# hyx1999/SAM-Decoding

Measured on AMD Instinct MI355X. Metric: tokens/sec (+ mean accepted tokens), Vicuna-7B bs=1, samd_sam_only draft+verify, higher is better.
Workload: dtype f16

## Files before the change

### sam-decoding_amd/csrc/verify_kernels.hip

```cpp
#include <hip/hip_runtime.h>
#include <hip/hip_fp16.h>
#include <cstdlib>
#include <cstring>
#include <vector>
#include "samd_common.h"
#include "topk_device.h"
#include "warm_device.h"

#define HIPCHK(x) do { hipError_t e_ = (x); if (e_ != hipSuccess) { samd_set_error("%s: %s", #x, hipGetErrorString(e_)); return SAMD_E_HIP; } } while (0)
#define LAUNCHCHK() do { hipError_t e_ = hipGetLastError(); if (e_ != hipSuccess) { samd_set_error("kernel launch: %s", hipGetErrorString(e_)); return SAMD_E_HIP; } } while (0)

typedef _Float16 half8 __attribute__((ext_vector_type(8)));
typedef __bf16 bf16x8 __attribute__((ext_vector_type(8)));
typedef float floatx4 __attribute__((ext_vector_type(4)));

struct F16 { typedef _Float16 elem; typedef half8 vec8; };
struct BF16 { typedef __bf16 elem; typedef bf16x8 vec8; };

__device__ __forceinline__ float to_f32(_Float16 x) { return (float)x; }
__device__ __forceinline__ float to_f32(__bf16 x) { return (float)x; }
__device__ __forceinline__ float to_f32(float x) { return x; }

template <typename T>
__global__ __launch_bounds__(1024) void k_argmax_rows(const T *__restrict__ logits, int rows, long long vocab, long long stride,
                                                      const int *__restrict__ d_rows, int *__restrict__ out) {
    const int row = blockIdx.x;
    if (d_rows && row >= d_rows[0]) return;
    if (row >= rows) return;
    const T *x = logits + (size_t)row * stride;
    float best = -INFINITY; long long bi = 0x7fffffffffffffffll;
    constexpr int VEC = 16 / sizeof(T);
    const bool vec_ok = ((((size_t)x) & 15) == 0);
    const long long nvec = vec_ok ? vocab / VEC : 0;
    for (long long c = threadIdx.x; c < nvec; c += blockDim.x) {
        const uint4 raw = reinterpret_cast<const uint4 *>(x)[c];
        const T *e = reinterpret_cast<const T *>(&raw);
#pragma unroll
        for (int j = 0; j < VEC; j++) {
            const float v = to_f32(e[j]); const long long i = c * VEC + j;
            if (v > best || (v == best && i < bi)) { best = v; bi = i; }
        }
    }
    for (long long i = nvec * VEC + threadIdx.x; i < vocab; i += blockDim.x) {
        const float v = to_f32(x[i]);
        if (v > best || (v == best && i < bi)) { best = v; bi = i; }
    }
    for (int o = 32; o > 0; o >>= 1) {
        const float ov = __shfl_xor(best, o); const long long oi = __shfl_xor(bi, o);
        if (ov > best || (ov == best && oi < bi)) { best = ov; bi = oi; }
    }
    __shared__ float sv[16]; __shared__ long long si[16];
    const int w = threadIdx.x >> 6;
    if ((threadIdx.x & 63) == 0) { sv[w] = best; si[w] = bi; }
    __syncthreads();
    if (threadIdx.x == 0) {
        const int nw = blockDim.x >> 6;
        for (int k = 1; k < nw; k++) if (sv[k] > best || (sv[k] == best && si[k] < bi)) { best = sv[k]; bi = si[k]; }
        out[row] = (bi == 0x7fffffffffffffffll) ? 0 : (int)bi;
    }
}

__global__ __launch_bounds__(256) void k_kv_compact(void *const *__restrict__ tensors, const int *__restrict__ verdict,
                                                    const int *__restrict__ kv_index, int n_heads, long long max_len, int row_bytes,
                                                    int h_start, int h_accept, int n_row_major) {
    extern __shared__ __attribute__((aligned(16))) unsigned char smem[];
    int a = h_accept, start = h_start;
    if (verdict) {
        if (!verdict[V_IS_TREE]) return;
        a = verdict[V_ACCEPT]; start = verdict[V_KV_START];
    }
    const int t = blockIdx.x / n_heads;
    unsigned char *base = (unsigned char *)tensors[t] + (size_t)(blockIdx.x % n_heads) * max_len * row_bytes;
    if (t >= n_row_major) {
        const int D = row_bytes >> 1, total = a * D;
        unsigned short *lds = reinterpret_cast<unsigned short *>(smem);
        unsigned short *col = reinterpret_cast<unsigned short *>(base);
        for (int c = threadIdx.x; c < total; c += blockDim.x) {
            const int d = c / a, j = c - d * a;
            lds[c] = col[(size_t)d * max_len + start + kv_index[j]];
        }
        __syncthreads();
        for (int c = threadIdx.x; c < total; c += blockDim.x) {
            const int d = c / a, j = c - d * a;
            if (kv_index[j] == j) continue;
            col[(size_t)d * max_len + start + j] = lds[c];
        }
        return;
    }
    const int chunks = row_bytes >> 4, total = a * chunks;
    uint4 *lds = reinterpret_cast<uint4 *>(smem);
    for (int c = threadIdx.x; c < total; c += blockDim.x) {
        const int j = c / chunks, k = c - j * chunks;
        const long long src = (long long)start + kv_index[j];
        lds[c] = reinterpret_cast<const uint4 *>(base + (size_t)src * row_bytes)[k];
    }
    __syncthreads();
    for (int c = threadIdx.x; c < total; c += blockDim.x) {
        const int j = c / chunks, k = c - j * chunks;
        if (kv_index[j] == j) continue;
        reinterpret_cast<uint4 *>(base + (size_t)(start + j) * row_bytes)[k] = lds[c];
    }
}

#define ATT_TILE 64
#define ATT_SPLITS 16
#define ATT_D 128
#define VT_STRIDE (ATT_TILE + 8)
#define P_STRIDE (ATT_TILE + 8)

template <typename TT> struct Mfma;
template <> struct Mfma<F16> {
    static __device__ __forceinline__ floatx4 run(half8 a, half8 b, floatx4 c) { return __builtin_amdgcn_mfma_f32_16x16x32_f16(a, b, c, 0, 0, 0); }
};
template <> struct Mfma<BF16> {
    static __device__ __forceinline__ floatx4 run(bf16x8 a, bf16x8 b, floatx4 c) { return __builtin_amdgcn_mfma_f32_16x16x32_bf16(a, b, c, 0, 0, 0); }
};

__device__ __forceinline__ int att_head_of_block(int bx, int n_heads) {
    return (n_heads & 7) == 0 ? (bx & 7) * (n_heads >> 3) + (bx >> 3) : bx;
}

template <typename TT, bool WIDE, bool VT = false>
__global__ __launch_bounds__(256) void k_tree_attention(const typename TT::elem *__restrict__ q, const typename TT::elem *__restrict__ kc,
                                                        const typename TT::elem *__restrict__ vc, float *__restrict__ ws,
                                                        int n_q_pad, int n_heads, int n_kv_heads, long long max_len,
                                                        const unsigned long long *__restrict__ mask, const int *__restrict__ d_L,
                                                        const int *__restrict__ d_n, float scale_log2, WarmArgs warm) {
    typedef typename TT::elem E;
    typedef typename TT::vec8 V8;
    __shared__ __attribute__((aligned(16))) E Vt[ATT_D * VT_STRIDE];
    __shared__ __attribute__((aligned(16))) E Pw[4 * 16 * P_STRIDE];

    const int h = att_head_of_block(blockIdx.x, n_heads), split = blockIdx.y;
    if (split >= ATT_SPLITS) {
        if (blockIdx.z != 0) return;
        const unsigned a = warm_next_projection(warm, (split - ATT_SPLITS) * n_heads + h);
        if (a == 0x9E3779B9u && n_q_pad < 0) ws[0] = 0.f;
        return;
    }
    const int tid = threadIdx.x, w = tid >> 6, l = tid & 63, lr = l & 15, lg = l >> 4;
    const int row_base = (WIDE ? 64 * (int)blockIdx.z : 0) + 16 * w;
    V8 qa[4];
    {
        const int qrow = row_base + lr;
        const E *qp = q + ((size_t)qrow * n_heads + h) * ATT_D + 8 * lg;
#pragma unroll
        for (int kk = 0; kk < 4; kk++) {
            uint4 raw = make_uint4(0, 0, 0, 0);
            if (qrow < n_q_pad) raw = *reinterpret_cast<const uint4 *>(qp + 32 * kk);
            qa[kk] = __builtin_bit_cast(V8, raw);
        }
    }
    unsigned long long mrow[4], mrow_hi[WIDE ? 4 : 1];
#pragma unroll
    for (int r = 0; r < 4; r++) {
        mrow[r] = mask[row_base + 4 * lg + r];
        if constexpr (WIDE) mrow_hi[r] = mask[SAMD_MAX_DRAFT + row_base + 4 * lg + r];
    }
    const int kvh = h / (n_heads / n_kv_heads);
    const E *kbase = kc + (size_t)kvh * max_len * ATT_D;
    const E *vbase = vc + (size_t)kvh * max_len * ATT_D;
    const bool may_be_active = row_base < n_q_pad;
    uint4 kraw[4][4], vra[2], vrb[2];
    auto load_k = [&](int key0) {
#pragma unroll
        for (int st = 0; st < 4; st++) {
            int key = key0 + 16 * st + lr;
// ... 3 lines not shown
            for (int kk = 0; kk < 4; kk++) kraw[st][kk] = *reinterpret_cast<const uint4 *>(kp + 32 * kk);
        }
    };
    auto load_v = [&](int key0) {
        if constexpr (VT) {
#pragma unroll
            for (int i = 0; i < 4; i++) {
                const int u = tid + 256 * i, d = u >> 3;
                int k0 = key0 + 8 * (u & 7);
                k0 = k0 + 8 <= (int)max_len ? k0 : (int)max_len - 8;
                const uint4 v = *reinterpret_cast<const uint4 *>(vbase + (size_t)d * max_len + k0);
                if (i == 0) vra[0] = v; else if (i == 1) vra[1] = v; else if (i == 2) vrb[0] = v; else vrb[1] = v;
            }
            return;
        }
#pragma unroll
        for (int it = 0; it < 2; it++) {
            const int p = tid >> 3, ch = (tid & 7) + 8 * it, d0 = 8 * ch;
            int ka = key0 + 2 * p, kb = ka + 1;
            ka = ka < (int)max_len ? ka : (int)max_len - 1; kb = kb < (int)max_len ? kb : (int)max_len - 1;
            vra[it] = *reinterpret_cast<const uint4 *>(vbase + (size_t)ka * ATT_D + d0);
            vrb[it] = *reinterpret_cast<const uint4 *>(vbase + (size_t)kb * ATT_D + d0);
        }
    };
    if (may_be_active) load_k(split * ATT_TILE);
    load_v(split * ATT_TILE);
    const int L = d_L[0];
    int n = d_n[0]; n = n > n_q_pad ? n_q_pad : n;
    const int total = L + n;
    const int ntiles = (total + ATT_TILE - 1) / ATT_TILE;
    if (split >= ntiles) return;
    const bool active = row_base < n;
#pragma unroll
    for (int r = 0; r < 4; r++) if (row_base + 4 * lg + r >= n) { mrow[r] = 0ull; if constexpr (WIDE) mrow_hi[r] = 0ull; }

    float m_run[4], l_run[4];
    floatx4 o[8];
#pragma unroll
    for (int r = 0; r < 4; r++) { m_run[r] = -INFINITY; l_run[r] = 0.f; }
#pragma unroll
    for (int dt = 0; dt < 8; dt++) o[dt] = (floatx4){0.f, 0.f, 0.f, 0.f};

    E *Pmine = Pw + w * 16 * P_STRIDE;

    for (int t = split; t < ntiles; t += ATT_SPLITS) {
        const int key0 = t * ATT_TILE;
        if (t != split && active) load_k(key0);
        __syncthreads();
        if (t != split) load_v(key0);
        if constexpr (VT) {
#pragma unroll
            for (int i = 0; i < 4; i++) {
                const int u = tid + 256 * i, d = u >> 3, kc8 = 8 * (u & 7);
                uint4 v = i == 0 ? vra[0] : (i == 1 ? vra[1] : (i == 2 ? vrb[0] : vrb[1]));
                const int live = total - key0 - kc8;
                if (live < 8) {
                    unsigned m[4];
#pragma unroll
                    for (int d2 = 0; d2 < 4; d2++) m[d2] = (2 * d2 < live ? 0xFFFFu : 0u) | (2 * d2 + 1 < live ? 0xFFFF0000u : 0u);
                    v.x &= m[0]; v.y &= m[1]; v.z &= m[2]; v.w &= m[3];
                }
                *reinterpret_cast<uint4 *>(&Vt[d * VT_STRIDE + kc8]) = v;
            }
        } else
#pragma unroll
        for (int it = 0; it < 2; it++) {
            const int p = tid >> 3, ch = (tid & 7) + 8 * it, d0 = 8 * ch;
            const int ka = key0 + 2 * p, kb = ka + 1;
            const uint4 ra = ka < total ? vra[it] : make_uint4(0, 0, 0, 0), rb = kb < total ? vrb[it] : make_uint4(0, 0, 0, 0);
            const unsigned short *ea = reinterpret_cast<const unsigned short *>(&ra);
            const unsigned short *eb = reinterpret_cast<const unsigned short *>(&rb);
#pragma unroll
            for (int j = 0; j < 8; j++)
                *reinterpret_cast<unsigned int *>(&Vt[(d0 + j) * VT_STRIDE + 2 * p]) = (unsigned int)ea[j] | ((unsigned int)eb[j] << 16);
        }
        floatx4 s[4];
        if (active) {
#pragma unroll
            for (int st = 0; st < 4; st++) {
                floatx4 acc = (floatx4){0.f, 0.f, 0.f, 0.f};
#pragma unroll
                for (int kk = 0; kk < 4; kk++) acc = Mfma<TT>::run(qa[kk], __builtin_bit_cast(V8, kraw[st][kk]), acc);
                s[st] = acc;
            }
            float tmax[4];
#pragma unroll
            for (int r = 0; r < 4; r++) tmax[r] = -INFINITY;
#pragma unroll
            for (int st = 0; st < 4; st++) {
                const int key = key0 + 16 * st + lr;
#pragma unroll
                for (int r = 0; r < 4; r++) {
                    const int rel = key - L;
                    bool ok;
                    if constexpr (WIDE) {
                        const unsigned long long word = rel < 64 ? mrow[r] : mrow_hi[r];
                        ok = (key < L) | ((key < total) & (bool)((word >> (rel & 63)) & 1ull));
                    } else ok = (key < L) | ((key < total) & (bool)((mrow[r] >> (rel & 63)) & 1ull));
                    const float v = ok ? s[st][r] * scale_log2 : -INFINITY;
                    s[st][r] = v;
                    tmax[r] = fmaxf(tmax[r], v);
                }
            }
#pragma unroll
            for (int r = 0; r < 4; r++) {
                const float v = row16_max(tmax[r]);
                const float m_new = fmaxf(m_run[r], v);
                const float m_use = m_new == -INFINITY ? 0.f : m_new;
                const float alpha = __builtin_amdgcn_exp2f(m_run[r] - m_use);
                float psum = 0.f;
#pragma unroll
                for (int st = 0; st < 4; st++) {
                    const float p = __builtin_amdgcn_exp2f(s[st][r] - m_use);
                    psum += p;
                    Pmine[(4 * lg + r) * P_STRIDE + 16 * st + lr] = (E)p;
                }
                psum = row16_sum(psum);
                l_run[r] = l_run[r] * alpha + psum;
                m_run[r] = m_new;
#pragma unroll
                for (int dt = 0; dt < 8; dt++) o[dt][r] *= alpha;
            }
        }
        __syncthreads();
        if (active) {
            V8 pa[2];
#pragma unroll
            for (int kcx = 0; kcx < 2; kcx++)
                pa[kcx] = __builtin_bit_cast(V8, *reinterpret_cast<const uint4 *>(&Pmine[lr * P_STRIDE + 32 * kcx + 8 * lg]));
#pragma unroll
            for (int dt = 0; dt < 8; dt++) {
#pragma unroll
                for (int kcx = 0; kcx < 2; kcx++) {
                    const uint4 raw = *reinterpret_cast<const uint4 *>(&Vt[(16 * dt + lr) * VT_STRIDE + 32 * kcx + 8 * lg]);
                    o[dt] = Mfma<TT>::run(pa[kcx], __builtin_bit_cast(V8, raw), o[dt]);
                }
            }
        }
    }
    if (active) {
#pragma unroll
        for (int r = 0; r < 4; r++) {
            const int row = row_base + 4 * lg + r;
            float *dst = ws + (((size_t)split * n_q_pad + row) * n_heads + h) * (ATT_D + 2);
            if (row < n_q_pad) {
#pragma unroll
                for (int dt = 0; dt < 8; dt++) dst[16 * dt + lr] = o[dt][r];
                if (lr == 0) { dst[ATT_D] = m_run[r]; dst[ATT_D + 1] = l_run[r]; }
            }
        }
    }
}

template <typename TT>
__global__ __launch_bounds__(64) void k_tree_attention_direct(const typename TT::elem *__restrict__ q, const typename TT::elem *__restrict__ kc,
                                                               const typename TT::elem *__restrict__ vt, float *__restrict__ ws,
                                                               int n_q_pad, int n_heads, int n_kv_heads, long long max_len,
                                                               const unsigned long long *__restrict__ mask, const int *__restrict__ d_L,
                                                               const int *__restrict__ d_n, float scale_log2, WarmArgs warm) {
    typedef typename TT::elem E;
    typedef typename TT::vec8 V8;
    __shared__ __attribute__((aligned(16))) E Pw[16 * P_STRIDE];
    const int h = att_head_of_block(blockIdx.x, n_heads), split = blockIdx.y;
    if (split >= ATT_SPLITS) {
        if (blockIdx.z != 0) return;
        const unsigned a = warm_next_projection(warm, (split - ATT_SPLITS) * n_heads + h);
        if (a == 0x9E3779B9u && n_q_pad < 0) ws[0] = 0.f;
        return;
    }
    const int l = threadIdx.x, lr = l & 15, lg = l >> 4;
    const int row_base = 16 * (int)blockIdx.z;
    V8 qa[4];
    {
        const E *qp = q + ((size_t)(row_base + lr) * n_heads + h) * ATT_D + 8 * lg;
#pragma unroll
        for (int kk = 0; kk < 4; kk++) {
            uint4 raw = make_uint4(0, 0, 0, 0);
            if (row_base + lr < n_q_pad) raw = *reinterpret_cast<const uint4 *>(qp + 32 * kk);
            qa[kk] = __builtin_bit_cast(V8, raw);
        }
    }
    unsigned long long mrow[4];
#pragma unroll
    for (int r = 0; r < 4; r++) mrow[r] = row_base + 4 * lg + r < n_q_pad ? mask[row_base + 4 * lg + r] : 0ull;
    const int kvh = h / (n_heads / n_kv_heads);
    const E *kbase = kc + (size_t)kvh * max_len * ATT_D;
    const E *vbase = vt + (size_t)kvh * max_len * ATT_D;
    uint4 kraw[4][4], vraw[8][2];
    auto load_kv = [&](int key0) {
#pragma unroll
        for (int st = 0; st < 4; st++) {
            int key = key0 + 16 * st + lr;
            key = key < (int)max_len ? key : (int)max_len - 1;
            const E *kp = kbase + (size_t)key * ATT_D + 8 * lg;
#pragma unroll
            for (int kk = 0; kk < 4; kk++) kraw[st][kk] = *reinterpret_cast<const uint4 *>(kp + 32 * kk);
        }
#pragma unroll
        for (int kcx = 0; kcx < 2; kcx++) {
            int k0 = key0 + 32 * kcx + 8 * lg;
            k0 = k0 + 8 <= (int)max_len ? k0 : (int)max_len - 8;
#pragma unroll
            for (int dt = 0; dt < 8; dt++) vraw[dt][kcx] = *reinterpret_cast<const uint4 *>(vbase + (size_t)(16 * dt + lr) * max_len + k0);
        }
    };
    load_kv(split * ATT_TILE);
    const int L = d_L[0];
    int n = d_n[0]; n = n > n_q_pad ? n_q_pad : n;
    const int total = L + n;
    const int ntiles = (total + ATT_TILE - 1) / ATT_TILE;
    if (split >= ntiles || row_base >= n) return;
#pragma unroll
    for (int r = 0; r < 4; r++) if (row_base + 4 * lg + r >= n) mrow[r] = 0ull;
    float m_run[4], l_run[4];
    floatx4 o[8];
#pragma unroll
    for (int r = 0; r < 4; r++) { m_run[r] = -INFINITY; l_run[r] = 0.f; }
#pragma unroll
    for (int dt = 0; dt < 8; dt++) o[dt] = (floatx4){0.f, 0.f, 0.f, 0.f};
    for (int t = split; t < ntiles; t += ATT_SPLITS) {
        const int key0 = t * ATT_TILE;
        if (t != split) load_kv(key0);
        floatx4 s[4];
#pragma unroll
        for (int st = 0; st < 4; st++) {
            floatx4 acc = (floatx4){0.f, 0.f, 0.f, 0.f};
#pragma unroll
            for (int kk = 0; kk < 4; kk++) acc = Mfma<TT>::run(qa[kk], __builtin_bit_cast(V8, kraw[st][kk]), acc);
            s[st] = acc;
        }
        float tmax[4];
#pragma unroll
        for (int r = 0; r < 4; r++) tmax[r] = -INFINITY;
#pragma unroll
        for (int st = 0; st < 4; st++) {
            const int key = key0 + 16 * st + lr;
#pragma unroll
            for (int r = 0; r < 4; r++) {
                const int rel = key - L;
                const bool ok = (key < L) | ((key < total) & (bool)((mrow[r] >> (rel & 63)) & 1ull));
                const float v = ok ? s[st][r] * scale_log2 : -INFINITY;
                s[st][r] = v;
                tmax[r] = fmaxf(tmax[r], v);
            }
        }
        if (t != split) { __builtin_amdgcn_fence(__ATOMIC_RELEASE, "wavefront"); __builtin_amdgcn_wave_barrier(); }
#pragma unroll
        for (int r = 0; r < 4; r++) {
            const float v = row16_max(tmax[r]);
            const float m_new = fmaxf(m_run[r], v);
            const float m_use = m_new == -INFINITY ? 0.f : m_new;
            const float alpha = __builtin_amdgcn_exp2f(m_run[r] - m_use);
            float psum = 0.f;
#pragma unroll
            for (int st = 0; st < 4; st++) {
                const float p = __builtin_amdgcn_exp2f(s[st][r] - m_use);
                psum += p;
                Pw[(4 * lg + r) * P_STRIDE + 16 * st + lr] = (E)p;
            }
            psum = row16_sum(psum);
            l_run[r] = l_run[r] * alpha + psum;
            m_run[r] = m_new;
#pragma unroll
            for (int dt = 0; dt < 8; dt++) o[dt][r] *= alpha;
        }
        if (key0 + ATT_TILE > total) {
#pragma unroll
            for (int kcx = 0; kcx < 2; kcx++) {
                const int live = total - key0 - 32 * kcx - 8 * lg;
                unsigned m[4];
#pragma unroll
                for (int d2 = 0; d2 < 4; d2++) m[d2] = (2 * d2 < live ? 0xFFFFu : 0u) | (2 * d2 + 1 < live ? 0xFFFF0000u : 0u);
#pragma unroll
                for (int dt = 0; dt < 8; dt++) { vraw[dt][kcx].x &= m[0]; vraw[dt][kcx].y &= m[1]; vraw[dt][kcx].z &= m[2]; vraw[dt][kcx].w &= m[3]; }
            }
        }
        __builtin_amdgcn_fence(__ATOMIC_RELEASE, "wavefront"); __builtin_amdgcn_wave_barrier();
        V8 pa[2];
#pragma unroll
        for (int kcx = 0; kcx < 2; kcx++) pa[kcx] = __builtin_bit_cast(V8, *reinterpret_cast<const uint4 *>(&Pw[lr * P_STRIDE + 32 * kcx + 8 * lg]));
#pragma unroll
        for (int dt = 0; dt < 8; dt++) {
#pragma unroll
            for (int kcx = 0; kcx < 2; kcx++) o[dt] = Mfma<TT>::run(pa[kcx], __builtin_bit_cast(V8, vraw[dt][kcx]), o[dt]);
        }
    }
#pragma unroll
    for (int r = 0; r < 4; r++) {
        const int row = row_base + 4 * lg + r;
        float *dst = ws + (((size_t)split * n_q_pad + row) * n_heads + h) * (ATT_D + 2);
        if (row < n) {
#pragma unroll
            for (int dt = 0; dt < 8; dt++) dst[16 * dt + lr] = o[dt][r];
            if (lr == 0) { dst[ATT_D] = m_run[r]; dst[ATT_D + 1] = l_run[r]; }
        }
    }
}

template <typename E>
__global__ __launch_bounds__(128) void k_attn_combine(const float *__restrict__ ws, E *__restrict__ out, int n_q_pad, int n_heads,
                                                      const int *__restrict__ d_L, const int *__restrict__ d_n, WarmArgs warm, int *__restrict__ arrive) {
    const int h = att_head_of_block(blockIdx.x, n_heads), row = blockIdx.y, d = threadIdx.x;
    if (row >= n_q_pad) {
        const unsigned a = warm_next_projection(warm, (row - n_q_pad) * n_heads + h);
        if (a == 0x9E3779B9u && n_q_pad < 0) out[0] = (E)0.f;
        return;
    }
    float mv[ATT_SPLITS], lv[ATT_SPLITS], pv[ATT_SPLITS];
    const int lane = d & 63;
    float2 ml = make_float2(-INFINITY, 0.f);
    if (lane < ATT_SPLITS) ml = *reinterpret_cast<const float2 *>(ws + (((size_t)lane * n_q_pad + row) * n_heads + h) * (ATT_D + 2) + ATT_D);
#pragma unroll
    for (int s = 0; s < ATT_SPLITS; s++) pv[s] = ws[(((size_t)s * n_q_pad + row) * n_heads + h) * (ATT_D + 2) + d];
#pragma unroll
    for (int s = 0; s < ATT_SPLITS; s++) { mv[s] = __shfl(ml.x, s); lv[s] = __shfl(ml.y, s); }
    int n = d_n[0]; n = n > n_q_pad ? n_q_pad : n;
    E *dst = out + ((size_t)row * n_heads + h) * ATT_D + d;
    float res = 0.f;
    if (row < n) {
        const int ntiles = (d_L[0] + n + ATT_TILE - 1) / ATT_TILE;
        const int used = ntiles < ATT_SPLITS ? ntiles : ATT_SPLITS;
        float M = -INFINITY;
#pragma unroll
        for (int s = 0; s < ATT_SPLITS; s++) if (s < used) M = fmaxf(M, mv[s]);
        float num = 0.f, den = 0.f;
#pragma unroll
        for (int s = 0; s < ATT_SPLITS; s++) {
            if (s >= used || mv[s] == -INFINITY) continue;
            const float wgt = exp2f(mv[s] - M);
            num += wgt * pv[s]; den += wgt * lv[s];
        }
        res = den > 0.f ? num / den : 0.f;
    }
    *dst = (E)res;
    if (arrive) {
        __syncthreads();
        if (threadIdx.x == 0) {
            __builtin_amdgcn_fence(__ATOMIC_RELEASE, "agent");
            asm volatile("s_waitcnt vmcnt(0)" ::: "memory");
            __hip_atomic_fetch_add(arrive, 1, __ATOMIC_RELAXED, __HIP_MEMORY_SCOPE_AGENT);
        }
    }
}

#define ATT_SLOTS (ATT_SPLITS + 1)
#define QS_STRIDE (ATT_D + 8)

template <typename TT, int NP>
__global__ __launch_bounds__(256, 2) void k_tree_attention_rope(const typename TT::elem *__restrict__ qkv, int n_part_rt, long long part_stride,
                                                               const float *__restrict__ cs, typename TT::elem *__restrict__ kc,
                                                               typename TT::elem *__restrict__ vc, float *__restrict__ ws,
                                                               int n_q_pad, int n_heads, int n_kv_heads, long long max_len,
                                                               const unsigned long long *__restrict__ mask, const int *__restrict__ d_L,
                                                               const int *__restrict__ d_n, float scale_log2) {
    typedef typename TT::elem E;
    typedef typename TT::vec8 V8;
    __shared__ __attribute__((aligned(16))) E Vt[ATT_D * VT_STRIDE];
    __shared__ __attribute__((aligned(16))) E Pw[4 * 16 * P_STRIDE];
    __shared__ __attribute__((aligned(16))) E Qs[ATT_TILE * QS_STRIDE];

    const int h = blockIdx.x, split = blockIdx.y;
    const bool fresh = split == ATT_SPLITS;
    const int tid = threadIdx.x, w = tid >> 6, l = tid & 63, lr = l & 15, lg = l >> 4;
    const int row_base = 16 * w;
    const int group = n_heads / n_kv_heads, kvh = h / group;
    const int W = (n_heads + 2 * n_kv_heads) * ATT_D;
    const float *part = reinterpret_cast<const float *>(qkv);

    auto ld4 = [&](size_t off, float (&x)[4]) {
        if constexpr (NP == 0) {
            const uint2 raw = *reinterpret_cast<const uint2 *>(qkv + off);
            const E *e = reinterpret_cast<const E *>(&raw);
#pragma unroll
            for (int i = 0; i < 4; i++) x[i] = (float)e[i];
        } else if constexpr (NP > 0) {
            float4 a[NP];
            const unsigned pst = (unsigned)part_stride;
#pragma unroll
            for (int k = 0; k < NP; k++) a[k] = *reinterpret_cast<const float4 *>(part + off + (unsigned)k * pst);
            float acc[4] = {0.f, 0.f, 0.f, 0.f};
#pragma unroll
            for (int k = 0; k < NP; k++) { acc[0] += a[k].x; acc[1] += a[k].y; acc[2] += a[k].z; acc[3] += a[k].w; }
#pragma unroll
            for (int i = 0; i < 4; i++) x[i] = (float)(E)acc[i];
        } else {
            float acc[4] = {0.f, 0.f, 0.f, 0.f};
            for (int k = 0; k < n_part_rt; k++) {
                const float4 a = *reinterpret_cast<const float4 *>(part + (size_t)k * part_stride + off);
                acc[0] += a.x; acc[1] += a.y; acc[2] += a.z; acc[3] += a.w;
            }
#pragma unroll
            for (int i = 0; i < 4; i++) x[i] = (float)(E)acc[i];
        }
    };
    auto rope_units = [&](int rows, int col0, E *dst, bool to_cache, const int *pL, const int *pn) {
        float x1[4][4], x2[4][4];
        float4 c[4], sn[4];
#pragma unroll
        for (int k = 0; k < 4; k++) {
            const int u = tid + 256 * k;
            if (u >= rows * 16) continue;
            const int r = u >> 4, e = 4 * (u & 15);
            ld4((size_t)r * W + col0 + e, x1[k]);
            ld4((size_t)r * W + col0 + e + 64, x2[k]);
            c[k] = *reinterpret_cast<const float4 *>(cs + r * ATT_D + e);
            sn[k] = *reinterpret_cast<const float4 *>(cs + r * ATT_D + 64 + e);
        }
        const int Lw = to_cache ? pL[0] : 0, nn = to_cache ? pn[0] : 0;
#pragma unroll
        for (int k = 0; k < 4; k++) {
            const int u = tid + 256 * k;
            if (u >= rows * 16) continue;
            const int r = u >> 4, e = 4 * (u & 15);
            const float cc[4] = {c[k].x, c[k].y, c[k].z, c[k].w}, ss[4] = {sn[k].x, sn[k].y, sn[k].z, sn[k].w};
            E lo[4], hi[4];
#pragma unroll
            for (int i = 0; i < 4; i++) {
                lo[i] = (E)(x1[k][i] * cc[i] - x2[k][i] * ss[i]);
// ... 394 lines not shown
        bool grown = false;
        while (true) {
            if (tid == 0) {
                int action = 0, tok = -1, hit = -1;
                while (row < C) {
                    const int j = row++;
                    bool eq = true;
                    for (int q = 0; q < n_acc; q++) eq = eq && cand[(size_t)j * D + q] == prefix[q];
                    if (!eq) continue;
                    const long long x = cand[(size_t)j * D + n_acc];
                    if (x < 0) continue;
                    bool dup = false;
                    for (int q = 0; q < n_seen && q < 1024; q++) dup = dup || seen[q] == (int)x;
                    if (dup) continue;
                    if (n_seen < 1024) seen[n_seen] = (int)x;
                    n_seen++;
                    if (k >= n_uniforms) { action = 3; break; }
                    const T r = (T)(float)uniforms[k++];
                    tok = (int)x; hit = j;
                    action = (float)r <= (float)work[tok] ? 1 : 2;
                    if (action == 1) prefix[n_acc] = x;
                    break;
                }
                s_action = action; s_tok = tok; s_row = hit;
            }
            __syncthreads();
            const int action = s_action, tok = s_tok;
            if (action == 0) break;
            if (action == 3) { status = 1; break; }
            if (action == 1) { best = s_row; n_acc++; grown = true; break; }
            if (tid == 0) work[tok] = (T)0.f;
            __syncthreads();
            float acc = 0.f;
            for (long long i = tid; i < V; i += blockDim.x) acc += (float)work[i];
            for (int o = 32; o > 0; o >>= 1) acc += __shfl_xor(acc, o);
            if ((tid & 63) == 0) red[tid >> 6] = acc;
            __syncthreads();
            float tot = 0.f;
            for (int w = 0; w < (int)(blockDim.x >> 6); w++) tot += red[w];
            const float denom = (float)(T)tot;
            for (long long i = tid; i < V; i += blockDim.x) work[i] = (T)((float)work[i] / denom);
            adjusted = 1;
            __syncthreads();
        }
        __syncthreads();
        if (!grown) break;
    }
    if (tid == 0) { out[0] = best; out[1] = n_acc; out[2] = k; out[3] = (adjusted && n_acc != D) ? 1 : 0; out[4] = status; }
}

extern "C" {

int samd_argmax_rows(const void *d_logits, int32_t dtype, int32_t rows, int64_t vocab, int64_t row_stride, const int32_t *d_rows,
                     int32_t *d_out, void *stream) {
    if (!d_logits || !d_out || rows < 0 || vocab < 1 || row_stride < vocab) { samd_set_error("samd_argmax_rows: invalid argument"); return SAMD_E_INVALID; }
    if (rows == 0) return SAMD_OK;
    hipStream_t st = (hipStream_t)stream;
    const int esz = dtype == SAMD_F32 ? 4 : 2;
    if ((row_stride * esz) % 16 != 0 && rows > 1) {
    }
    switch (dtype) {
    case SAMD_F16: hipLaunchKernelGGL(k_argmax_rows<_Float16>, dim3(rows), dim3(1024), 0, st, (const _Float16 *)d_logits, rows, (long long)vocab, (long long)row_stride, d_rows, d_out); break;
    case SAMD_BF16: hipLaunchKernelGGL(k_argmax_rows<__bf16>, dim3(rows), dim3(1024), 0, st, (const __bf16 *)d_logits, rows, (long long)vocab, (long long)row_stride, d_rows, d_out); break;
    case SAMD_F32: hipLaunchKernelGGL(k_argmax_rows<float>, dim3(rows), dim3(1024), 0, st, (const float *)d_logits, rows, (long long)vocab, (long long)row_stride, d_rows, d_out); break;
    default: samd_set_error("samd_argmax_rows: bad dtype"); return SAMD_E_INVALID;
    }
    LAUNCHCHK();
    return SAMD_OK;
}

static int kv_compact(samd_session_t *s, void *const *d_tensors, int32_t n_tensors, int32_t n_transposed, int32_t n_heads, int64_t max_len,
                      int32_t head_dim, int32_t elem_bytes, int32_t start, const int32_t *d_indices, int32_t accept, void *stream) {
    if (!d_tensors || n_tensors < 1 || n_transposed < 0 || n_transposed > n_tensors || n_heads < 1 || head_dim < 1 || (head_dim * elem_bytes) % 16 != 0 ||
        (n_transposed > 0 && elem_bytes != 2)) {
        samd_set_error("samd_kv_compact: invalid argument (row bytes must be a multiple of 16; transposed tensors hold 2-byte elements)"); return SAMD_E_INVALID;
    }
    const int row_bytes = head_dim * elem_bytes;
    const size_t lds = (size_t)SAMD_MAX_DRAFT * row_bytes;
    if (lds > 64 * 1024) { samd_set_error("samd_kv_compact: row too large"); return SAMD_E_INVALID; }
    if (s) hipLaunchKernelGGL(k_kv_compact, dim3(n_tensors * n_heads), dim3(256), lds, (hipStream_t)stream, d_tensors, s->dev.verdict, s->dev.kv_index, n_heads,
                              (long long)max_len, row_bytes, 0, 0, n_tensors - n_transposed);
    else hipLaunchKernelGGL(k_kv_compact, dim3(n_tensors * n_heads), dim3(256), lds, (hipStream_t)stream, d_tensors, (const int *)nullptr, d_indices, n_heads,
                            (long long)max_len, row_bytes, start, accept, n_tensors - n_transposed);
    LAUNCHCHK();
    return SAMD_OK;
}

int samd_posterior_sampled(const void *d_probs, int32_t dtype, const int64_t *d_candidates, int32_t n_candidates, int32_t depth, int64_t vocab,
                           const double *d_uniforms, int32_t n_uniforms, void *d_work, int32_t *d_out, void *stream) {
    return samd_posterior_sampled_nodes(d_probs, dtype, nullptr, 0, d_candidates, n_candidates, depth, vocab, d_uniforms, n_uniforms, d_work, d_out, stream);
}

int samd_posterior_sampled_nodes(const void *d_probs, int32_t dtype, const int32_t *d_rowmap, int32_t n_rows, const int64_t *d_candidates, int32_t n_candidates,
                                 int32_t depth, int64_t vocab, const double *d_uniforms, int32_t n_uniforms, void *d_work, int32_t *d_out, void *stream) {
    if (!d_probs || !d_candidates || n_candidates < 1 || depth < 1 || depth > SAMD_MAX_DRAFT || vocab < 1 || !d_uniforms || n_uniforms < 0 || !d_work || !d_out ||
        (d_rowmap && n_rows < 1)) {
        samd_set_error("samd_posterior_sampled: invalid argument (depth <= 128)"); return SAMD_E_INVALID;
    }
    hipStream_t st = (hipStream_t)stream;
    if (dtype == SAMD_F32) hipLaunchKernelGGL(k_posterior_sampled<float>, dim3(1), dim3(1024), 0, st, (const float *)d_probs, (const long long *)d_candidates, n_candidates, depth,
                                              (long long)vocab, d_uniforms, n_uniforms, (float *)d_work, d_out, d_rowmap, n_rows);
    else if (dtype == SAMD_F16) hipLaunchKernelGGL(k_posterior_sampled<_Float16>, dim3(1), dim3(1024), 0, st, (const _Float16 *)d_probs, (const long long *)d_candidates, n_candidates,
                                                   depth, (long long)vocab, d_uniforms, n_uniforms, (_Float16 *)d_work, d_out, d_rowmap, n_rows);
    else if (dtype == SAMD_BF16) hipLaunchKernelGGL(k_posterior_sampled<__bf16>, dim3(1), dim3(1024), 0, st, (const __bf16 *)d_probs, (const long long *)d_candidates, n_candidates,
                                                    depth, (long long)vocab, d_uniforms, n_uniforms, (__bf16 *)d_work, d_out, d_rowmap, n_rows);
    else { samd_set_error("samd_posterior_sampled: bad dtype"); return SAMD_E_INVALID; }
    LAUNCHCHK();
    return SAMD_OK;
}

int samd_kv_compact(samd_session_t *s, void *const *d_tensors, int32_t n_tensors, int32_t n_heads, int64_t max_len,
                    int32_t head_dim, int32_t elem_bytes, void *stream) {
    if (!s) { samd_set_error("samd_kv_compact: null session"); return SAMD_E_INVALID; }
    return kv_compact(s, d_tensors, n_tensors, 0, n_heads, max_len, head_dim, elem_bytes, 0, nullptr, 0, stream);
}

int samd_kv_compact_indices(void *const *d_tensors, int32_t n_tensors, int32_t n_heads, int64_t max_len, int32_t head_dim,
                            int32_t elem_bytes, int32_t start, const int32_t *d_indices, int32_t accept, void *stream) {
    if (!d_indices || start < 0 || accept < 0 || accept > SAMD_MAX_DRAFT || start + accept > max_len) { samd_set_error("samd_kv_compact_indices: invalid argument"); return SAMD_E_INVALID; }
    if (accept == 0) return SAMD_OK;
    return kv_compact(nullptr, d_tensors, n_tensors, 0, n_heads, max_len, head_dim, elem_bytes, start, d_indices, accept, stream);
}

int samd_kv_compact_vt(samd_session_t *s, void *const *d_tensors, int32_t n_tensors, int32_t n_transposed, int32_t n_heads, int64_t max_len,
                       int32_t head_dim, int32_t elem_bytes, void *stream) {
    if (!s) { samd_set_error("samd_kv_compact_vt: null session"); return SAMD_E_INVALID; }
    return kv_compact(s, d_tensors, n_tensors, n_transposed, n_heads, max_len, head_dim, elem_bytes, 0, nullptr, 0, stream);
}

int samd_kv_compact_indices_vt(void *const *d_tensors, int32_t n_tensors, int32_t n_transposed, int32_t n_heads, int64_t max_len, int32_t head_dim,
                               int32_t elem_bytes, int32_t start, const int32_t *d_indices, int32_t accept, void *stream) {
    if (!d_indices || start < 0 || accept < 0 || accept > SAMD_MAX_DRAFT || start + accept > max_len) { samd_set_error("samd_kv_compact_indices_vt: invalid argument"); return SAMD_E_INVALID; }
    if (accept == 0) return SAMD_OK;
    return kv_compact(nullptr, d_tensors, n_tensors, n_transposed, n_heads, max_len, head_dim, elem_bytes, start, d_indices, accept, stream);
}

int64_t samd_tree_attention_workspace(int32_t n_q_pad, int32_t n_heads, int32_t head_dim) {
    return (int64_t)ATT_SPLITS * n_q_pad * n_heads * (head_dim + 2) * 4;
}

int samd_tree_attention(const void *d_q, const void *d_k_cache, const void *d_v_cache, void *d_out, int32_t dtype, int32_t n_q_pad,
                        int32_t n_heads, int32_t n_kv_heads, int32_t head_dim, int64_t max_len, const uint64_t *d_mask,
                        const int32_t *d_cache_length, const int32_t *d_n, float scale, void *d_workspace, int64_t workspace_bytes,
                        void *stream) {
    return samd_tree_attention_warm(d_q, d_k_cache, d_v_cache, d_out, dtype, n_q_pad, n_heads, n_kv_heads, head_dim, max_len, d_mask, d_cache_length, d_n,
                                    scale, d_workspace, workspace_bytes, nullptr, stream);
}

static int att_direct_rows() {
    static const int rows = [] { const char *e = getenv("SAMD_ATT_DIRECT_ROWS"); const int r = e ? atoi(e) : 16; return r < 0 ? 0 : (r > 64 ? 64 : r); }();
    return rows;
}

static int tree_attention_impl(const void *d_q, const void *d_k_cache, const void *d_v_cache, void *d_out, int32_t dtype, int32_t n_q_pad,
                               int32_t n_heads, int32_t n_kv_heads, int32_t head_dim, int64_t max_len, const uint64_t *d_mask,
                               const int32_t *d_cache_length, const int32_t *d_n, float scale, void *d_workspace, int64_t workspace_bytes,
                               const samd_warm_t *next, int *d_arrive, void *stream, int v_transposed = 0) {
    if (v_transposed && (max_len < 8 || max_len % 8 != 0)) { samd_set_error("samd_tree_attention_vt: max_len must be a multiple of 8"); return SAMD_E_INVALID; }
    const WarmArgs none = warm_args(nullptr);
    const WarmArgs wa_split = next && next->where == 0 ? warm_args(next) : none, wa = next && next->where != 0 ? warm_args(next) : none;
    const int warm_rows = (warm_blocks(wa) + n_heads - 1) / n_heads;
    const int warm_splits = (warm_blocks(wa_split) + n_heads - 1) / n_heads;
    if (!d_q || !d_k_cache || !d_v_cache || !d_out || !d_mask || !d_cache_length || !d_n || !d_workspace) { samd_set_error("samd_tree_attention: null pointer"); return SAMD_E_INVALID; }
    if (head_dim != ATT_D || n_q_pad < 1 || n_q_pad > SAMD_MAX_DRAFT || n_heads < 1 || n_kv_heads < 1 || n_heads % n_kv_heads != 0 ||
        (dtype != SAMD_F16 && dtype != SAMD_BF16) || workspace_bytes < samd_tree_attention_workspace(n_q_pad, n_heads, head_dim)) {
        samd_set_error("samd_tree_attention: unsupported shape (head_dim must be 128, n_q_pad <= 128, f16/bf16) or workspace too small");
        return SAMD_E_INVALID;
    }
    const int row_tiles = (n_q_pad + 63) / 64;
    hipStream_t st = (hipStream_t)stream;
    const float scale_log2 = scale * 1.4426950408889634f;
    float *ws = (float *)d_workspace;
#define ATT_GO(TT, ET, W) if (v_transposed && n_q_pad <= att_direct_rows()) \
                          hipLaunchKernelGGL((k_tree_attention_direct<TT>), dim3(n_heads, ATT_SPLITS + warm_splits, (n_q_pad + 15) / 16), dim3(64), 0, st, (const ET *)d_q, \
                           (const ET *)d_k_cache, (const ET *)d_v_cache, ws, n_q_pad, n_heads, n_kv_heads, (long long)max_len, \
                           (const unsigned long long *)d_mask, d_cache_length, d_n, scale_log2, wa_split); \
                      else if (v_transposed) hipLaunchKernelGGL((k_tree_attention<TT, W, true>), dim3(n_heads, ATT_SPLITS + warm_splits, row_tiles), dim3(256), 0, st, (const ET *)d_q, \
                           (const ET *)d_k_cache, (const ET *)d_v_cache, ws, n_q_pad, n_heads, n_kv_heads, (long long)max_len, \
                           (const unsigned long long *)d_mask, d_cache_length, d_n, scale_log2, wa_split); \
                      else hipLaunchKernelGGL((k_tree_attention<TT, W>), dim3(n_heads, ATT_SPLITS + warm_splits, row_tiles), dim3(256), 0, st, (const ET *)d_q, \
                           (const ET *)d_k_cache, (const ET *)d_v_cache, ws, n_q_pad, n_heads, n_kv_heads, (long long)max_len, \
                           (const unsigned long long *)d_mask, d_cache_length, d_n, scale_log2, wa_split)
    if (dtype == SAMD_F16) {
        if (row_tiles > 1) { ATT_GO(F16, _Float16, true); } else { ATT_GO(F16, _Float16, false); }
        hipLaunchKernelGGL(k_attn_combine<_Float16>, dim3(n_heads, n_q_pad + warm_rows), dim3(ATT_D), 0, st, ws, (_Float16 *)d_out, n_q_pad, n_heads, d_cache_length, d_n, wa, d_arrive);
    } else {
        if (row_tiles > 1) { ATT_GO(BF16, __bf16, true); } else { ATT_GO(BF16, __bf16, false); }
        hipLaunchKernelGGL(k_attn_combine<__bf16>, dim3(n_heads, n_q_pad + warm_rows), dim3(ATT_D), 0, st, ws, (__bf16 *)d_out, n_q_pad, n_heads, d_cache_length, d_n, wa, d_arrive);
    }
#undef ATT_GO
    LAUNCHCHK();
    return SAMD_OK;
}

int samd_tree_attention_warm(const void *d_q, const void *d_k_cache, const void *d_v_cache, void *d_out, int32_t dtype, int32_t n_q_pad,
                             int32_t n_heads, int32_t n_kv_heads, int32_t head_dim, int64_t max_len, const uint64_t *d_mask,
                             const int32_t *d_cache_length, const int32_t *d_n, float scale, void *d_workspace, int64_t workspace_bytes,
                             const samd_warm_t *next, void *stream) {
    return tree_attention_impl(d_q, d_k_cache, d_v_cache, d_out, dtype, n_q_pad, n_heads, n_kv_heads, head_dim, max_len, d_mask, d_cache_length, d_n, scale,
                               d_workspace, workspace_bytes, next, nullptr, stream);
}

int samd_tree_attention_vt(const void *d_q, const void *d_k_cache, const void *d_vt_cache, void *d_out, int32_t dtype, int32_t n_q_pad,
                           int32_t n_heads, int32_t n_kv_heads, int32_t head_dim, int64_t max_len, const uint64_t *d_mask,
                           const int32_t *d_cache_length, const int32_t *d_n, float scale, void *d_workspace, int64_t workspace_bytes,
                           const samd_warm_t *next, void *stream) {
    return tree_attention_impl(d_q, d_k_cache, d_vt_cache, d_out, dtype, n_q_pad, n_heads, n_kv_heads, head_dim, max_len, d_mask, d_cache_length, d_n, scale,
                               d_workspace, workspace_bytes, next, nullptr, stream, 1);
}

int samd_tree_attention_signal(const void *d_q, const void *d_k_cache, const void *d_v_cache, void *d_out, int32_t dtype, int32_t n_q_pad,
                               int32_t n_heads, int32_t n_kv_heads, int32_t head_dim, int64_t max_len, const uint64_t *d_mask,
                               const int32_t *d_cache_length, const int32_t *d_n, float scale, void *d_workspace, int64_t workspace_bytes,
                               int32_t *d_arrive, void *stream) {
    if (!d_arrive) return SAMD_E_INVALID;
    return tree_attention_impl(d_q, d_k_cache, d_v_cache, d_out, dtype, n_q_pad, n_heads, n_kv_heads, head_dim, max_len, d_mask, d_cache_length, d_n, scale,
                               d_workspace, workspace_bytes, nullptr, d_arrive, stream);
}

int64_t samd_tree_attention_rope_workspace(int32_t n_q_pad, int32_t n_heads, int32_t head_dim) {
    return (int64_t)ATT_SLOTS * n_q_pad * n_heads * (head_dim + 2) * 4;
}

int samd_tree_attention_rope(const void *d_qkv, int32_t n_partials, int64_t partial_stride, const float *d_cs, void *d_k_cache, void *d_v_cache,
                             void *d_out, int32_t dtype, int32_t n_q_pad, int32_t n_heads, int32_t n_kv_heads, int32_t head_dim, int64_t max_len,
                             const uint64_t *d_mask, const int32_t *d_cache_length, const int32_t *d_n, float scale, void *d_workspace,
                             int64_t workspace_bytes, void *stream) {
    if (!d_qkv || !d_cs || !d_k_cache || !d_v_cache || !d_out || !d_mask || !d_cache_length || !d_n || !d_workspace) { samd_set_error("samd_tree_attention_rope: null pointer"); return SAMD_E_INVALID; }
    if (head_dim != ATT_D || n_q_pad < 1 || n_q_pad > 64 || n_heads < 1 || n_kv_heads < 1 || n_heads % n_kv_heads != 0 || n_partials < 0 ||
        (dtype != SAMD_F16 && dtype != SAMD_BF16) || workspace_bytes < samd_tree_attention_rope_workspace(n_q_pad, n_heads, head_dim)) {
        samd_set_error("samd_tree_attention_rope: unsupported shape (head_dim must be 128, n_q_pad <= 64, f16/bf16) or workspace too small");
        return SAMD_E_INVALID;
    }
    hipStream_t st = (hipStream_t)stream;
    const float scale_log2 = scale * 1.4426950408889634f;
    float *ws = (float *)d_workspace;
#define GO(TT, NP, ET) hipLaunchKernelGGL((k_tree_attention_rope<TT, NP>), dim3(n_heads, ATT_SLOTS), dim3(256), 0, st, (const ET *)d_qkv, n_partials, (long long)partial_stride, \
        d_cs, (ET *)d_k_cache, (ET *)d_v_cache, ws, n_q_pad, n_heads, n_kv_heads, (long long)max_len, (const unsigned long long *)d_mask, d_cache_length, d_n, scale_log2)
#define GO2(TT, ET) do { if (n_partials == 0) GO(TT, 0, ET); else if (n_partials == 2) GO(TT, 2, ET); else if (n_partials == 5) GO(TT, 5, ET); else GO(TT, -1, ET); \
        hipLaunchKernelGGL(k_attn_combine_slots<ET>, dim3(n_q_pad, n_heads), dim3(ATT_D), 0, st, ws, (ET *)d_out, n_q_pad, n_heads, d_cache_length, d_n); } while (0)
    if (dtype == SAMD_F16) GO2(F16, _Float16); else GO2(BF16, __bf16);
#undef GO2
#undef GO
    LAUNCHCHK();
    return SAMD_OK;
}

int samd_recycle_create(int32_t vocab, const int32_t *h_child_offsets, const int32_t *h_children, int32_t n_nodes, samd_recycle_t **out) {
    if (!out || vocab < 1 || n_nodes < 1 || n_nodes > SAMD_MAX_DRAFT || !h_child_offsets) { samd_set_error("samd_recycle_create: invalid argument"); return SAMD_E_INVALID; }
    int ndev = 0;
    if (hipGetDeviceCount(&ndev) != hipSuccess || ndev < 1) { samd_set_error("no HIP device"); return SAMD_E_NODEVICE; }
    std::vector<int> parent(n_nodes, -1), depth(n_nodes, 0);
    const int n_child = h_child_offsets[n_nodes];
    for (int i = 0; i < n_nodes; i++)
        for (int c = h_child_offsets[i]; c < h_child_offsets[i + 1]; c++) {
            const int ch = h_children[c];
            if (ch <= i || ch >= n_nodes || (c - h_child_offsets[i]) >= SAMD_TOPK) { samd_set_error("samd_recycle_create: bad tree"); return SAMD_E_INVALID; }
            parent[ch] = i;
        }
    int n_levels = 1;
    for (int i = 1; i < n_nodes; i++) { depth[i] = parent[i] < 0 ? 0 : depth[parent[i]] + 1; n_levels = std::max(n_levels, depth[i] + 1); }
    std::vector<int> level_off(n_levels + 1, 0), level_nodes(n_nodes);
    for (int i = 0; i < n_nodes; i++) level_off[depth[i] + 1]++;
    for (int lv = 0; lv < n_levels; lv++) level_off[lv + 1] += level_off[lv];
    { std::vector<int> fill(level_off.begin(), level_off.end() - 1); for (int i = 0; i < n_nodes; i++) level_nodes[fill[depth[i]]++] = i; }

    samd_recycle_t *t = (samd_recycle_t *)calloc(1, sizeof(samd_recycle_t));
    if (!t) { samd_set_error("out of host memory"); return SAMD_E_CAPACITY; }
    t->vocab = vocab; t->n_nodes = n_nodes; t->n_levels = n_levels; t->tmp_rows = 16384;
    bool ok = hipMalloc((void **)&t->d_table, (size_t)vocab * 8 * 4) == hipSuccess;
    ok = ok && hipMalloc((void **)&t->d_present, (size_t)vocab) == hipSuccess;
    ok = ok && hipMalloc((void **)&t->d_tmp, (size_t)t->tmp_rows * 8 * 4) == hipSuccess;
    t->n_split = (vocab + E2_SEG - 1) / E2_SEG;
    if (t->n_split > E2_MAXSPLIT) t->n_split = 0;
    if (t->n_split) {
        ok = ok && hipMalloc((void **)&t->d_part_v, (size_t)t->tmp_rows * t->n_split * E2_K * 4) == hipSuccess;
        ok = ok && hipMalloc((void **)&t->d_part_i, (size_t)t->tmp_rows * t->n_split * E2_K * 4) == hipSuccess;
    }
    ok = ok && hipMalloc((void **)&t->d_child_off, (n_nodes + 1) * 4) == hipSuccess;
    ok = ok && hipMalloc((void **)&t->d_children, std::max(1, n_child) * 4) == hipSuccess;
    ok = ok && hipMalloc((void **)&t->d_level_off, (n_levels + 1) * 4) == hipSuccess;
    ok = ok && hipMalloc((void **)&t->d_level_nodes, n_nodes * 4) == hipSuccess;
    ok = ok && hipMemset(t->d_table, 0, (size_t)vocab * 8 * 4) == hipSuccess && hipMemset(t->d_present, 0, (size_t)vocab) == hipSuccess;
    ok = ok && hipMemcpy(t->d_child_off, h_child_offsets, (n_nodes + 1) * 4, hipMemcpyHostToDevice) == hipSuccess;
    if (n_child) ok = ok && hipMemcpy(t->d_children, h_children, n_child * 4, hipMemcpyHostToDevice) == hipSuccess;
    ok = ok && hipMemcpy(t->d_level_off, level_off.data(), (n_levels + 1) * 4, hipMemcpyHostToDevice) == hipSuccess;
    ok = ok && hipMemcpy(t->d_level_nodes, level_nodes.data(), n_nodes * 4, hipMemcpyHostToDevice) == hipSuccess;
    if (!ok) { samd_recycle_free(t); samd_set_error("samd_recycle_create: device allocation failed"); return SAMD_E_HIP; }
    *out = t;
    return SAMD_OK;
}

void samd_recycle_free(samd_recycle_t *t) {
    if (!t) return;
    void *ptrs[] = { t->d_table, t->d_present, t->d_tmp, t->d_part_v, t->d_part_i, t->d_child_off, t->d_children, t->d_level_off, t->d_level_nodes };
    for (void *p : ptrs) if (p) (void)hipFree(p);
    free(t);
}

int samd_recycle_update(samd_recycle_t *t, const int32_t *d_tokens, const void *d_logits, int32_t dtype, int32_t n, const int32_t *d_n,
                        int64_t vocab, int64_t row_stride, void *stream) {
    if (!t || !d_tokens || !d_logits || n < 0 || n > t->tmp_rows || vocab < 8 || vocab > t->vocab) { samd_set_error("samd_recycle_update: invalid argument"); return SAMD_E_INVALID; }
    if (n == 0) return SAMD_OK;
    hipStream_t st = (hipStream_t)stream;
    const int n_split = t->n_split ? (int)((vocab + E2_SEG - 1) / E2_SEG) : 0;
    if (n_split && (dtype == SAMD_F16 || dtype == SAMD_BF16)) {
        const dim3 grid(n, n_split);
        if (dtype == SAMD_F16) hipLaunchKernelGGL(k_topk8_part<_Float16>, grid, dim3(256), 0, st, (const _Float16 *)d_logits, n, (long long)vocab, (long long)row_stride, d_n, n_split, t->d_part_v, t->d_part_i);
        else hipLaunchKernelGGL(k_topk8_part<__bf16>, grid, dim3(256), 0, st, (const __bf16 *)d_logits, n, (long long)vocab, (long long)row_stride, d_n, n_split, t->d_part_v, t->d_part_i);
        hipLaunchKernelGGL(k_topk8_merge, dim3(n), dim3(256), 0, st, n, d_n, n_split, (const float *)t->d_part_v, (const int *)t->d_part_i, t->d_tmp);
    } else
    switch (dtype) {
    case SAMD_F16: hipLaunchKernelGGL(k_topk8_rows<_Float16>, dim3(n), dim3(256), 0, st, (const _Float16 *)d_logits, n, (long long)vocab, (long long)row_stride, d_n, t->d_tmp); break;
    case SAMD_BF16: hipLaunchKernelGGL(k_topk8_rows<__bf16>, dim3(n), dim3(256), 0, st, (const __bf16 *)d_logits, n, (long long)vocab, (long long)row_stride, d_n, t->d_tmp); break;
    case SAMD_F32: hipLaunchKernelGGL(k_topk8_rows<float>, dim3(n), dim3(256), 0, st, (const float *)d_logits, n, (long long)vocab, (long long)row_stride, d_n, t->d_tmp); break;
    default: return SAMD_E_INVALID;
    }
    hipLaunchKernelGGL(k_recycle_scatter, dim3((n + 255) / 256), dim3(256), 0, st, d_tokens, t->d_tmp, n, d_n, t->d_table, t->d_present, t->vocab);
    LAUNCHCHK();
    return SAMD_OK;
}

int samd_recycle_draft(samd_recycle_t *t, const int32_t *d_start_token, int32_t *d_out, void *stream) {
    if (!t || !d_start_token || !d_out) return SAMD_E_INVALID;
    hipLaunchKernelGGL(k_recycle_draft, dim3(1), dim3(64), 0, (hipStream_t)stream, t->d_table, t->d_present, t->vocab, t->d_child_off,
                       t->d_children, t->d_level_off, t->d_level_nodes, t->n_nodes, t->n_levels, d_start_token, d_out);
    LAUNCHCHK();
// ... 13 lines not shown
```

Baseline: 826.1.

## Stage K/V tiles through LDS with async global_load_lds and swizzled layout

Adds a LINES variant of the direct tree-attention kernel that copies each K and V tile straight into swizzled shared-memory images using global_load_lds. Fragments are then read back with ds_read_b128, and hand-placed waitcnt instructions let the V loads overlap the QK MFMA and softmax. The aim is to replace strided per-lane register loads with coalesced line loads and to hide V latency. The variant is on by default and can be turned off with an env var. In exchange it uses about 32KB of LDS per 64-thread block, which may lower occupancy, and it depends on fragile manual waitcnt counts.

```diff
diff --git a/sam-decoding_amd/csrc/verify_kernels.hip b/sam-decoding_amd/csrc/verify_kernels.hip
--- a/sam-decoding_amd/csrc/verify_kernels.hip
+++ b/sam-decoding_amd/csrc/verify_kernels.hip
@@ -13,6 +13,8 @@
 typedef _Float16 half8 __attribute__((ext_vector_type(8)));
 typedef __bf16 bf16x8 __attribute__((ext_vector_type(8)));
 typedef float floatx4 __attribute__((ext_vector_type(4)));
+typedef __attribute__((address_space(1))) const void *gptr_t;
+typedef __attribute__((address_space(3))) void *lptr_t;
 
 struct F16 { typedef _Float16 elem; typedef half8 vec8; };
 struct BF16 { typedef __bf16 elem; typedef bf16x8 vec8; };
@@ -322,7 +324,7 @@
     }
 }
 
-template <typename TT>
+template <typename TT, bool LINES>
 __global__ __launch_bounds__(64) void k_tree_attention_direct(const typename TT::elem *__restrict__ q, const typename TT::elem *__restrict__ kc,
                                                                const typename TT::elem *__restrict__ vt, float *__restrict__ ws,
                                                                int n_q_pad, int n_heads, int n_kv_heads, long long max_len,
@@ -331,6 +333,8 @@
     typedef typename TT::elem E;
     typedef typename TT::vec8 V8;
     __shared__ __attribute__((aligned(16))) E Pw[16 * P_STRIDE];
+    __shared__ __attribute__((aligned(16))) E Kimg[LINES ? ATT_TILE * ATT_D : 8];
+    __shared__ __attribute__((aligned(16))) E Vimg[LINES ? ATT_D * ATT_TILE : 8];
     const int h = att_head_of_block(blockIdx.x, n_heads), split = blockIdx.y;
     if (split >= ATT_SPLITS) {
         if (blockIdx.z != 0) return;
@@ -358,6 +362,27 @@
     const E *vbase = vt + (size_t)kvh * max_len * ATT_D;
     uint4 kraw[4][4], vraw[8][2];
     auto load_kv = [&](int key0) {
+        if constexpr (LINES) {
+#pragma unroll
+            for (int i = 0; i < 16; i++) {
+                const int kl = 4 * i + lg, unit = lr ^ (kl & 15);
+                int key = key0 + kl;
+                key = key < (int)max_len ? key : (int)max_len - 1;
+                const char *src = reinterpret_cast<const char *>(kbase) + (uint32_t)(key * (ATT_D * 2) + 16 * unit);
+                __builtin_amdgcn_global_load_lds((gptr_t)src, (lptr_t)(Kimg + 512 * i), 16, 0, 0);
+                asm volatile("" ::: "memory");
+            }
+#pragma unroll
+            for (int j = 0; j < 16; j++) {
+                const int d = 8 * j + (l >> 3), piece = (l & 7) ^ ((d >> 1) & 7);
+                int k0 = key0 + 8 * piece;
+                k0 = k0 + 8 <= (int)max_len ? k0 : (int)max_len - 8;
+                const char *src = reinterpret_cast<const char *>(vbase) + (uint32_t)(2 * (d * (int)max_len + k0));
+                __builtin_amdgcn_global_load_lds((gptr_t)src, (lptr_t)(Vimg + 512 * j), 16, 0, 0);
+                asm volatile("" ::: "memory");
+            }
+            return;
+        }
 #pragma unroll
         for (int st = 0; st < 4; st++) {
             int key = key0 + 16 * st + lr;
@@ -374,7 +399,31 @@
             for (int dt = 0; dt < 8; dt++) vraw[dt][kcx] = *reinterpret_cast<const uint4 *>(vbase + (size_t)(16 * dt + lr) * max_len + k0);
         }
     };
-    load_kv(split * ATT_TILE);
+    auto read_k = [&]() {
+        typedef unsigned u32x4 __attribute__((ext_vector_type(4)));
+        asm volatile("s_waitcnt vmcnt(16)" ::: "memory");
+        const uint32_t kb = (uint32_t)(uintptr_t)(lptr_t)Kimg + (uint32_t)lr * (ATT_D * 2);
+#pragma unroll
+        for (int kk = 0; kk < 4; kk++) {
+            const uint32_t a = kb + (uint32_t)((4 * kk + lg) ^ lr) * 16;
+            u32x4 r0, r1, r2, r3;
+            asm volatile("ds_read_b128 %0, %4\n\tds_read_b128 %1, %4 offset:4096\n\tds_read_b128 %2, %4 offset:8192\n\tds_read_b128 %3, %4 offset:12288"
+                         : "=&v"(r0), "=&v"(r1), "=&v"(r2), "=&v"(r3) : "v"(a));
+            kraw[0][kk] = __builtin_bit_cast(uint4, r0); kraw[1][kk] = __builtin_bit_cast(uint4, r1);
+            kraw[2][kk] = __builtin_bit_cast(uint4, r2); kraw[3][kk] = __builtin_bit_cast(uint4, r3);
+        }
+        asm volatile("s_waitcnt lgkmcnt(0)" ::: "memory");
+        __builtin_amdgcn_sched_barrier(0);
+    };
+    auto read_v = [&]() {
+        asm volatile("s_waitcnt vmcnt(0)" ::: "memory");
+#pragma unroll
+        for (int dt = 0; dt < 8; dt++)
+#pragma unroll
+            for (int kcx = 0; kcx < 2; kcx++)
+                vraw[dt][kcx] = *reinterpret_cast<const uint4 *>(Vimg + (16 * dt + lr) * ATT_TILE + 8 * ((4 * kcx + lg) ^ (lr >> 1)));
+    };
+    if constexpr (!LINES) load_kv(split * ATT_TILE);
     const int L = d_L[0];
     int n = d_n[0]; n = n > n_q_pad ? n_q_pad : n;
     const int total = L + n;
@@ -382,6 +431,11 @@
     if (split >= ntiles || row_base >= n) return;
 #pragma unroll
     for (int r = 0; r < 4; r++) if (row_base + 4 * lg + r >= n) mrow[r] = 0ull;
+    if constexpr (LINES) {
+#pragma unroll
+        for (int r = 0; r < 4; r++) asm volatile("" : "+v"(mrow[r]) : : "memory");
+        load_kv(split * ATT_TILE);
+    }
     float m_run[4], l_run[4];
     floatx4 o[8];
 #pragma unroll
@@ -390,7 +444,11 @@
     for (int dt = 0; dt < 8; dt++) o[dt] = (floatx4){0.f, 0.f, 0.f, 0.f};
     for (int t = split; t < ntiles; t += ATT_SPLITS) {
         const int key0 = t * ATT_TILE;
-        if (t != split) load_kv(key0);
+        if (t != split) {
+            if constexpr (LINES) asm volatile("s_waitcnt lgkmcnt(0)" ::: "memory");
+            load_kv(key0);
+        }
+        if constexpr (LINES) read_k();
         floatx4 s[4];
 #pragma unroll
         for (int st = 0; st < 4; st++) {
@@ -434,6 +492,7 @@
 #pragma unroll
             for (int dt = 0; dt < 8; dt++) o[dt][r] *= alpha;
         }
+        if constexpr (LINES) read_v();
         if (key0 + ATT_TILE > total) {
 #pragma unroll
             for (int kcx = 0; kcx < 2; kcx++) {
@@ -1134,6 +1193,11 @@
     return rows;
 }
 
+static bool att_lines() {
+    const char *e = getenv("SAMD_ATT_LINES");
+    return e ? atoi(e) != 0 : true;
+}
+
 static int tree_attention_impl(const void *d_q, const void *d_k_cache, const void *d_v_cache, void *d_out, int32_t dtype, int32_t n_q_pad,
                                int32_t n_heads, int32_t n_kv_heads, int32_t head_dim, int64_t max_len, const uint64_t *d_mask,
                                const int32_t *d_cache_length, const int32_t *d_n, float scale, void *d_workspace, int64_t workspace_bytes,
@@ -1154,7 +1218,8 @@
     const float scale_log2 = scale * 1.4426950408889634f;
     float *ws = (float *)d_workspace;
 #define ATT_GO(TT, ET, W) if (v_transposed && n_q_pad <= att_direct_rows()) \
-                          hipLaunchKernelGGL((k_tree_attention_direct<TT>), dim3(n_heads, ATT_SPLITS + warm_splits, (n_q_pad + 15) / 16), dim3(64), 0, st, (const ET *)d_q, \
+                          hipLaunchKernelGGL((att_lines() && max_len <= (1 << 22) ? k_tree_attention_direct<TT, true> : k_tree_attention_direct<TT, false>),  \
+                           dim3(n_heads, ATT_SPLITS + warm_splits, (n_q_pad + 15) / 16), dim3(64), 0, st, (const ET *)d_q, \
                            (const ET *)d_k_cache, (const ET *)d_v_cache, ws, n_q_pad, n_heads, n_kv_heads, (long long)max_len, \
                            (const unsigned long long *)d_mask, d_cache_length, d_n, scale_log2, wa_split); \
                       else if (v_transposed) hipLaunchKernelGGL((k_tree_attention<TT, W, true>), dim3(n_heads, ATT_SPLITS + warm_splits, row_tiles), dim3(256), 0, st, (const ET *)d_q, \
```

Result: no change. 828.4, median of 6 (+0.3%).
